# hkust-vgd/scanobjectnn

Measured on AMD Instinct MI355X. Metric: point-clouds/sec fwd+bwd at B×2048×3, 15-cls, higher is better.
Workload: dtype f32

## Files before the change

include/pcops.h:

```cpp
#ifndef PCOPS_H
#define PCOPS_H

#ifdef __cplusplus
extern "C" {
#endif

typedef void *pcops_stream_t;

typedef struct pcops_rows {
    const void *blocks;
    const int *block_start;
    const int *rows;
} pcops_rows_t;

typedef enum pcops_status {
    PCOPS_OK = 0,
    PCOPS_ERR_NULL_POINTER = -1,
    PCOPS_ERR_BAD_SHAPE = -2,
    PCOPS_ERR_BAD_ARGUMENT = -3,
    PCOPS_ERR_UNSUPPORTED = -4,
    PCOPS_ERR_LAUNCH = -5
} pcops_status;

const char *pcops_strerror(int status);
// ... 131 lines not shown
int pcops_mlp_wgrad_splits(long long M, int K, int N);
int pcops_mlp_wgrad(long long M, int K, int N, const float *X, int ldx, const float *a_scale,
                    const float *a_shift, const float *G, const float *Y, const float *p, const float *q,
                    const float *t, const float *gpool, const unsigned char *argmax, int S,
                    const float *pool_scale, const float *pool_shift, float *partial, float *dW, float *db,
                    pcops_stream_t stream);
int pcops_mlp_transpose(int K, int N, const float *W, float *Wt, pcops_stream_t stream);
int pcops_mlp_bwd_fused_groups(long long M, int K, int N, int S, int pooled);
int pcops_mlp_bwd_fused(long long M, int K, int N, const float *Yprev, const float *a_scale, const float *a_shift,
                        const float *G, const float *Y, const float *p, const float *q, const float *t,
                        const float *gpool, const unsigned char *argmax, int S, const float *W, float *partial,
                        float *dW, float *db, float *Gprev, float *stats_partial, pcops_stream_t stream);
int pcops_mlp_bwd_fused_rows(long long M, int K, int N, const float *Yprev, const float *a_scale, const float *a_shift,
                             const float *G, const float *Y, const float *p, const float *q, const float *t,
                             const float *gpool, const unsigned char *argmax, int S, const float *W, float *partial,
                             float *dW, float *db, float *Gprev, float *stats_partial, const pcops_rows_t *rows,
                             pcops_stream_t stream);
int pcops_mlp_dy_apply(long long M, int N, const float *G, const float *Y, const float *p, const float *q, const float *t,
                       float *out, pcops_stream_t stream);
int pcops_small_gemm(int M, int K, int N, const float *A, int lda, const float *B, int ldb, float *C, int ldc,
                     pcops_stream_t stream);
int pcops_small_gemm_ex(int M, int K, int N, const float *A, int lda, int transA, const float *B, int ldb, int transB,
                        const float *bias, float *C, int ldc, pcops_stream_t stream);
int pcops_small_gemm_colsum(int M, int K, int N, const float *A, int lda, int transA, const float *B, int ldb, int transB,
                            const float *bias, float *C, int ldc, float *colsum, pcops_stream_t stream);
typedef struct pcops_gemm_problem {
    int M, K, N;
    const float *A; int lda, transA;
    const float *B; int ldb, transB;
    const float *bias;
    float *C; int ldc;
    float *colsum;
} pcops_gemm_problem_t;
int pcops_small_gemm_pair(const pcops_gemm_problem_t *p, pcops_stream_t stream);

int pcops_mlp_pool_top_supported(int M, int Kp, int N, int S);
int pcops_mlp_pool_top_prep(int Kp, int N, const float *W, const float *b, const float *q, const float *t, float *Wt,
                            float *Wq, float *u, float *v, pcops_stream_t stream);
int pcops_mlp_pool_top_finish(int Kp, int N, long long M, float *dW, const float *Ssp, const float *xsum, const float *u,
                              const float *cfsum, const float *q, const float *W, const float *b, const float *t,
                              float *db, pcops_stream_t stream);
int pcops_mlp_pool_top_addend(int M, int Kp, int N, int S, const float *gout, const float *ysel,
                            const unsigned char *argmax, const float *pool_scale, const float *pool_shift,
                            const float *p, const float *Wt, float *addend, int *rowmap, pcops_stream_t stream);
int pcops_mlp_gemm_dgrad_top(int M, int Kp, const float *Yprev, const float *prev_scale, const float *prev_shift,
                             const float *Mq, const float *vconst, const float *addend, long long addend_rows,
                             const int *rowmap, float *Gprev, float *stats_partial, pcops_stream_t stream);
int pcops_mlp_gram(long long M, int Kp, const float *Yprev, int ldx, const float *a_scale, const float *a_shift,
                   float *partial, float *gram, float *xsum, pcops_stream_t stream);
int pcops_mlp_pool_top_wsparse(int M, int Kp, int N, int S, const float *gout, const float *ysel,
                               const unsigned char *argmax, const float *pool_scale, const float *pool_shift,
                               const float *p, const float *Yprev, const float *prev_scale, const float *prev_shift,
                               float *Ssp, float *cfsum, pcops_stream_t stream);
int pcops_mlp_xyz_supported(int M, int C1, int N2);
int pcops_mlp_bwd_fused_xyz_rows(long long M, int K, int N, const float *off4, const float *xyzw, const float *a_scale,
                                 const float *a_shift, const float *G, const float *Y, const float *p, const float *q,
                                 const float *t, const float *gpool, const unsigned char *argmax, int S, const float *W,
                                 float *partial, float *dW, float *db, float *stats_partial, float *xyz_stats,
                                 const pcops_rows_t *rows, pcops_stream_t stream);
int pcops_mlp_gemm_fwd_xyz(int M, int K, int N, const float *off4, const float *xyzw, const float *pro_scale,
                           const float *pro_shift, const float *W, const float *bias, float *Y,
                           float *stats_partial, const float *stat_pivot, pcops_stream_t stream);
int pcops_mlp_gemm_dgrad_xyz(int M, int K, int Nout, const float *G, const float *Y, const float *p,
                             const float *q, const float *t, const float *gpool, const unsigned char *argmax,
                             int S, const float *pool_scale, const float *pool_shift, const float *Wt,
                             const float *off4, const float *xyzw, const float *prev_scale,
                             const float *prev_shift, float *Gprev, float *stats_partial, float *xyz_stats,
                             pcops_stream_t stream);
int pcops_mlp_wgrad_xyz(long long M, int K, int N, const float *off4, const float *xyzw, const float *a_scale,
                        const float *a_shift, const float *G, const float *Y, const float *p, const float *q,
                        const float *t, const float *gpool, const unsigned char *argmax, int S,
                        const float *pool_scale, const float *pool_shift, float *partial, float *dW, float *db,
                        pcops_stream_t stream);

int pcops_sa_gather_stats_rows(long long groups);
int pcops_sa_gather_fwd_stats_rows(int b, int n, int m, int s, int c, int has_q, int has_ctr, int other_terms,
                                   int compacted);
int pcops_sa_gather_fwd(int b, int n, int m, int s, int c, const float *Q, const float *Ctr, const float *xyz,
                        const float *new_xyz, const float *Wxyz, const float *bias, const int *idx, float *Y,
                        float *off4, float *stats_partial, const float *stat_pivot, float *moments,
                        pcops_stream_t stream);
int pcops_sa_scatter_rows(int b, int m);
unsigned long long pcops_sa_scatter_workspace_bytes(int b, int n, int m, int s);
int pcops_sa_scatter_bwd(int b, int n, int m, int s, int c, const float *G, const float *Y, const float *p,
                         const float *q, const float *t, const float *gpool, const unsigned char *argmax,
                         const float *pool_scale, const float *pool_shift, const int *idx, const float *xyz,
                         const float *new_xyz, float *dQ, float *dCtr, float *wpartial, float *dWxyz,
                         float *dbias, const float *fwd_Q, const float *fwd_Ctr, const float *fwd_Wxyz,
                         const float *fwd_bias, void *workspace, pcops_stream_t stream);

int pcops_edge_pool_stats_rows(long long groups);
int pcops_edge_pool_fwd_stats_rows(int b, int n, int m, int s, int c);
int pcops_edge_pool_fwd(int b, int n, int m, int s, int c, const float *Q, const float *Ctr, const int *idx,
                        const float *gamma, float *SQ, float *qsel, unsigned char *arg, float *stats_partial,
                        const float *stat_pivot, pcops_stream_t stream);
int pcops_edge_pool_out(long long groups, int c, const float *qsel, const float *Ctr, const float *scale,
                        const float *shift, float *out, float *ysel, pcops_stream_t stream);
int pcops_edge_pool_bwd(int b, int n, int m, int s, int c, const float *Q, const float *Ctr, const int *idx,
                        const float *gpool, const float *ysel, const float *SQ, const unsigned char *arg,
                        const float *scale, const float *shift, const float *p, const float *q, const float *t,
                        float *dQ, float *dCtr, void *workspace, pcops_stream_t stream);
int pcops_cloud_bias_supported(long long rows, int rows_per_group, int c);
int pcops_cloud_bias_rows(long long rows);
int pcops_cloud_bias_fwd(long long rows, int rows_per_group, int c, const float *Q, const float *Ctr, float *Y,
                         float *stats_partial, const float *stat_pivot, pcops_stream_t stream);
int pcops_cloud_bias_bwd(long long rows, int rows_per_group, int c, const float *G, const float *Y, const float *p, const float *q,
// ... 223 lines not shown
```

scanobjectnn_amd/fused_mlp.py:

```python
import os
from collections import namedtuple
from typing import NamedTuple, Optional, Tuple

import torch

from . import _lib
from . import dist as _dist


def _f32(n, dev):
    return torch.empty(n, dtype=torch.float32, device=dev)


class _VecArena:

    def __init__(self, widths, per_width, dev):
        total = sum(((n + 3) // 4 * 4) * per_width for n in widths)
        alloc = torch.empty if all(n % 4 == 0 for n in widths) else torch.zeros
        self.buf = alloc(total, dtype=torch.float32, device=dev)
        self.off = 0

    def take(self, n):
        n4 = (n + 3) // 4 * 4
        v = self.buf[self.off:self.off + n4]
        self.off += n4
        return v


def _workspace(n, dev):
    lib = _lib.load()
    return torch.empty(int(lib.pcops_mlp_reduce_workspace_bytes(n)) // 8, dtype=torch.float64, device=dev)


def _p(t):
    return t.data_ptr() if t is not None else None


F_QC, F_CLOUD, F_GATHER, F_XYZ, F_POOL_ROWS, F_ROWS, F_POOL, F_GEMM = (
    "qc", "cloud_bias", "gather", "xyz", "pool_rows", "rows", "pool", "gemm")
F_CLOUD_POINT = "cloud_point"
B_XYZ_FIRST, B_EDGE_FIRST, B_QC, B_CLOUD, B_SCATTER, B_SCATTER_ID = (
    "xyz_first", "edge_first", "qc_scatter", "cloud_bias", "scatter", "scatter_identity")
B_CLOUD_POINT = "cloud_point"
B_TOP, B_SPLIT, B_SPLIT_XYZ = "top", "split", "split_xyz"
B_ONEPASS, B_ONEPASS_XYZ, B_ONEPASS_GW, B_ONEPASS_EDGE, B_ONEPASS_EDGE_GW = (
    "onepass", "onepass_xyz", "onepass_gw", "onepass_edge", "onepass_edge_gw")
_ONEPASS = (B_ONEPASS, B_ONEPASS_XYZ, B_ONEPASS_GW, B_ONEPASS_EDGE, B_ONEPASS_EDGE_GW)
_READS_Y = (B_CLOUD, B_CLOUD_POINT, B_SCATTER, B_SCATTER_ID, B_SPLIT, B_SPLIT_XYZ) + _ONEPASS
_READS_Y_BELOW = (B_TOP, B_SPLIT, B_ONEPASS, B_ONEPASS_GW, B_ONEPASS_EDGE, B_ONEPASS_EDGE_GW)


class LayerPlan(NamedTuple):
    fwd: str
    K: Optional[int]
    N: int
    store_y: bool
    pooled: str
    bwd: str
    count: int


class StackPlan(NamedTuple):
    virt: bool
    rows: bool
    direct: bool
    edge_rows: bool
    need_dx: bool
    tail_fold: bool
    layers: Tuple[LayerPlan, ...]

    @property
    def pool_top(self):
        return self.layers[-1].bwd == B_TOP


def plan_stack(*, R, S, K0, widths, pool, training, need_grad, need_dx, sync, w_aligned, has_b, geom=None, present=(),
               a0_contiguous=True, rows=False, point_k=None):
    lib = _lib.load()
    L, C1 = len(widths), widths[0]
    point = bool(pool & 16)
    identity, qc, direct, pool = bool(pool & 2), bool(pool & 4), bool(pool & 8), bool(pool & 1)
    gather = geom is not None
    direct = gather and qc and direct
    virt = (gather and "a0" not in present and "ctr" not in present and "wxyz" in present
            and (L >= 3 or (L == 2 and not pool)) and not sync and (training or not need_grad)
            and bool(lib.pcops_mlp_xyz_supported(R, C1, widths[1])))
    rows = rows and not (gather and "a0" not in present and not virt)
    edge_rows = False
    layers = []
    for l, N in enumerate(widths):
        K = widths[l - 1] if l else K0
        top = pool and l == L - 1
        store_y, pooled, bwd, count = True, "", "", 0
        onepass = int(need_grad and BWD_FUSED and l > 0 and lib.pcops_mlp_bwd_fused_groups(R, K, N, S if top else 0, int(top)))
        if l == 0 and gather:
            B, Nsrc, M = geom
            if point:
                if not (gather and identity and not qc and CLOUD_POINT_FUSED and set(present) == {"a0", "ctr", "wxyz"}
                        and not rows and not top and M == 1 and Nsrc == S and a0_contiguous and point_k is not None
                        and lib.pcops_cloud_point_supported(B, S, point_k, C1)):
                    raise _lib.PcopsError("plan_stack: no per-cloud + per-point first layer for this stack")
                fwd = F_CLOUD_POINT
            elif qc:
                fwd = F_QC
            elif (identity and CLOUD_BIAS and set(present) == {"a0", "ctr"} and not rows and M == 1 and Nsrc == S
                    and a0_contiguous and lib.pcops_cloud_bias_supported(R, S, C1)):
                fwd = F_CLOUD
            else:
                fwd, store_y = F_GATHER, not virt
            if need_grad:
                shortcut = "a0" in present and need_dx and identity and not top
                bwd = (B_CLOUD_POINT if fwd == F_CLOUD_POINT else B_XYZ_FIRST if virt else B_EDGE_FIRST if direct
                       else B_QC if qc else B_CLOUD if (fwd == F_CLOUD and not top) else B_SCATTER_ID if shortcut else B_SCATTER)
        else:
            xyz_prev = virt and l == 1
            algebraic = False
            if xyz_prev:
                fwd = F_XYZ
            elif rows and top and l > 0 and FUSE_POOL_ROWS and lib.pcops_mlp_gemm_fwd_pool_rows_supported(R, K, N):
                fwd, pooled = F_POOL_ROWS, "rows"
                algebraic = bool(need_grad and POOL_TOP and POOL_TOP_ROWS and S >= 64 and N >= 2 * K and has_b[l]
                                 and not onepass and lib.pcops_mlp_pool_top_rows_supported(R, K, N, S))
                store_y = not algebraic
            elif rows:
                fwd = F_ROWS
            elif top and lib.pcops_mlp_gemm_fwd_pool_supported(R, K, N, S):
                fwd, pooled = F_POOL, "raw"
                algebraic = bool(need_grad and POOL_TOP and S >= 64 and N >= 2 * K and has_b[l]
                                 and lib.pcops_mlp_pool_top_supported(R, K, N, S))
                store_y = need_grad and not algebraic
            else:
                fwd = F_GEMM
            if algebraic:
                bwd, count = B_TOP, lib.pcops_mlp_wgrad_splits(R, K, K)
            elif onepass and w_aligned[l]:
                use_edge = (direct and top and l == 1 and EDGE_DIRECT_FUSED
                            and lib.pcops_mlp_bwd_fused_edge_groups(R, K, N, S, 0) == onepass)
                gw = (top and not rows and not xyz_prev and
                      (lib.pcops_mlp_bwd_fused_edge_groups(R, K, N, S, 1) if use_edge
                       else lib.pcops_mlp_bwd_fused_gw_groups(R, K, N, S)) == onepass)
                edge_rows = edge_rows or use_edge
                bwd = ((B_ONEPASS_EDGE_GW if gw else B_ONEPASS_EDGE) if use_edge else B_ONEPASS_GW if gw
                       else B_ONEPASS_XYZ if xyz_prev else B_ONEPASS)
                count = onepass
            elif need_grad:
                bwd, count = (B_SPLIT_XYZ if xyz_prev else B_SPLIT), lib.pcops_mlp_wgrad_splits(R, K, N)
        layers.append(LayerPlan(fwd, K, N, bool(store_y), pooled, bwd, int(count)))
    for l, lp in enumerate(layers):
        reads = (lp.bwd in _READS_Y or (l + 1 < L and layers[l + 1].bwd in _READS_Y_BELOW)
                 or (need_grad and not pool and l == L - 1))
        assert lp.store_y or not reads, (l, layers)
    return StackPlan(bool(virt), bool(rows), direct, bool(edge_rows), bool(need_dx), TAIL_FOLD, tuple(layers))


StackSaved = namedtuple("StackSaved", "a0 ctr idx xyz new_xyz wxyz bias Ys means rstds scales shifts Ws gammas argmax ysel "
                                      "off4 xyzw mom")


def _bn_forward(bn, N, R, P, part, piv, *, training, sync, need_grad, hyper, vecs, ws):
    (gamma, beta, mm, mv), (eps, decay, unbiased) = bn, hyper
    scale, shift = vecs.take(N), vecs.take(N)
    mean = rstd = None
    if training:
        mean, rstd = vecs.take(N), vecs.take(N)
        Pf, Rf, piv_fin = P, R, piv
        if sync:
            part, Rf = _dist.allreduce_stat_partials(part, R, mm if piv is not None else None)
            Pf, piv_fin = part.shape[0], None
        _lib.call("pcops_mlp_bn_finalize", Pf, N, Rf, part.data_ptr(), piv_fin, ws.data_ptr(), gamma.data_ptr(),
                  beta.data_ptr(), float(eps), float(decay), int(unbiased), mm.data_ptr(), mv.data_ptr(),
                  mean.data_ptr(), rstd.data_ptr(), scale.data_ptr(), shift.data_ptr())
    else:
        _lib.call("pcops_mlp_bn_eval_coeffs", N, gamma.data_ptr(), beta.data_ptr(), mm.data_ptr(),
                  mv.data_ptr(), float(eps), scale.data_ptr(), shift.data_ptr())
        if need_grad:
            mean, rstd = mm.detach().clone(), torch.rsqrt(mv.detach() + float(eps))
    return scale, shift, mean, rstd


def _bn_backward(N, R, P, part, gamma, mean, rstd, *, training, sync, vecs, ws):
    dev = part.device
    dgamma, dbeta = _f32(N, dev), _f32(N, dev)
    p, q, t = vecs.take(N), vecs.take(N), vecs.take(N)
    _lib.call("pcops_mlp_bn_bwd_coeffs", P, N, R, part.data_ptr(), ws.data_ptr(), gamma.data_ptr(),
              mean.data_ptr(), rstd.data_ptr(), dgamma.data_ptr(), dbeta.data_ptr(),
              p.data_ptr(), q.data_ptr(), t.data_ptr())
    if sync:
        gpart, Rg = _dist.allreduce_stat_partials(part, R)
        junk = _f32(2 * N, dev)
        _lib.call("pcops_mlp_bn_bwd_coeffs", gpart.shape[0], N, Rg, gpart.data_ptr(), ws.data_ptr(), gamma.data_ptr(),
                  mean.data_ptr(), rstd.data_ptr(), junk.data_ptr(), junk[N:].data_ptr(),
                  p.data_ptr(), q.data_ptr(), t.data_ptr())
    if not training:
        q.zero_()
        t.zero_()
    return dgamma, dbeta, p, q, t


class FusedMLPStack(torch.autograd.Function):

# ... 419 lines not shown
                  S, psc, psh, scratch.data_ptr(), dW.data_ptr(), db.data_ptr(), rref)
    else:
        src, asc, ash = (sv.Ys[l - 1], sv.scales[l - 1].data_ptr(), sv.shifts[l - 1].data_ptr()) if l else (sv.a0, None, None)
        _lib.call("pcops_mlp_wgrad_rows", R, K, N, src.data_ptr(), K, asc, ash, Gptr, Y.data_ptr(),
                  p.data_ptr(), q.data_ptr(), t.data_ptr(), gp, am, S, psc, psh, scratch.data_ptr(),
                  dW.data_ptr(), db.data_ptr(), rref)
    dn.grads[6 * l + 0] = dW
    dn.grads[6 * l + 1] = db
    if l == 0 and not dn.plan.need_dx:
        return
    Wt = _f32((N, K), dev)
    _lib.call("pcops_mlp_transpose", K, N, sv.Ws[l].data_ptr(), Wt.data_ptr())
    Gprev = None if xyz_prev else _f32((R, K), dev)
    if l > 0:
        dn.P = lib.pcops_mlp_stats_rows(R)
        dn.part = _f32((dn.P, 2, K), dev)
    if xyz_prev:
        dn.xstats = _f32((dn.P, 3, K), dev)
        _lib.call("pcops_mlp_gemm_dgrad_xyz_rows", R, N, K, Gptr, Y.data_ptr(), p.data_ptr(), q.data_ptr(),
                  t.data_ptr(), gp, am, S, psc, psh, Wt.data_ptr(), sv.off4.data_ptr(), sv.xyzw.data_ptr(),
                  sv.scales[0].data_ptr(), sv.shifts[0].data_ptr(), None, dn.part.data_ptr(), dn.xstats.data_ptr(),
                  rref)
    elif l > 0:
        _lib.call("pcops_mlp_gemm_dgrad_rows", R, N, K, Gptr, Y.data_ptr(), p.data_ptr(), q.data_ptr(),
                  t.data_ptr(), gp, am, S, psc, psh, Wt.data_ptr(), sv.Ys[l - 1].data_ptr(),
                  sv.scales[l - 1].data_ptr(), sv.shifts[l - 1].data_ptr(), Gprev.data_ptr(),
                  dn.part.data_ptr(), rref)
    else:
        _lib.call("pcops_mlp_gemm_dgrad", R, N, K, Gptr, Y.data_ptr(), p.data_ptr(), q.data_ptr(),
                  t.data_ptr(), gp, am, S, psc, psh, Wt.data_ptr(), None, None, None,
                  Gprev.data_ptr(), None)
    dn.Gm = Gprev


def _pool_top_backward(dn, l, lp, p, q, t):
    lib = _lib.load()
    sv, dev, R, S, rows, rref = dn.sv, dn.dev, dn.R, dn.S, dn.rows, dn.rref
    K, N, fold = lp.K, lp.N, dn.plan.tail_fold
    W, b, grad_out = sv.Ws[l], dn.biases[l].detach(), dn.grad_out
    ysel, argmax, sc, sh = sv.ysel, sv.argmax, sv.scales[l], sv.shifts[l]
    Yprev, psc, psh = (sv.Ys[l - 1], sv.scales[l - 1], sv.shifts[l - 1]) if l > 0 else (sv.a0, None, None)
    need_dx = l > 0 or dn.plan.need_dx
    Wt = _f32((N, K), dev)
    if fold:
        Wq, u = _f32((K, N), dev), _f32(N, dev)
        v = _f32(K, dev) if need_dx else None
        _lib.call("pcops_mlp_pool_top_prep", K, N, W.data_ptr(), b.data_ptr(), q.data_ptr(), t.data_ptr(), Wt.data_ptr(),
                  Wq.data_ptr(), u.data_ptr(), _p(v))
    else:
        _lib.call("pcops_mlp_transpose", K, N, W.data_ptr(), Wt.data_ptr())
        Wq = W * q[:N]
        u = torch.addcmul(t[:N], q[:N], b)
    Gprev = part = None
    scratch = _f32(lp.count * (K * K + K), dev)
    gram, xsum = _f32((K, K), dev), _f32(K, dev)
    if rows is not None:
        _lib.call("pcops_mlp_gram_rows", R, K, Yprev.data_ptr(), K, _p(psc), _p(psh), scratch.data_ptr(),
                  gram.data_ptr(), xsum.data_ptr(), rref)
    else:
        _lib.call("pcops_mlp_gram", R, K, Yprev.data_ptr(), K, _p(psc), _p(psh), scratch.data_ptr(),
                  gram.data_ptr(), xsum.data_ptr())
    dW = _f32((K, N), dev)
    paired = fold and need_dx
    if paired:
        Mq = _f32((K, K), dev)
        _lib.small_gemm_pair((K, N, K, Wq.data_ptr(), N, 0, Wt.data_ptr(), K, 0, None, Mq.data_ptr(), K, None),
                             (K, K, N, gram.data_ptr(), K, 0, Wq.data_ptr(), N, 0, None, dW.data_ptr(), N, None))
    if need_dx:
        if not paired:
            Mq = _f32((K, K), dev)
            _lib.call("pcops_small_gemm", K, N, K, Wq.data_ptr(), N, Wt.data_ptr(), K, Mq.data_ptr(), K)
        if not fold:
            v = _f32(K, dev)
            _lib.call("pcops_small_gemm", 1, N, K, u.data_ptr(), N, Wt.data_ptr(), K, v.data_ptr(), K)
        G = R // S
        addend = _f32((R if rows is not None else G * min(S, N), K), dev)
        rowmap = torch.empty(R, dtype=torch.int32, device=dev)
        Gprev = _f32((R, K), dev)
        part = _f32((lib.pcops_mlp_stats_rows(R), 2, K), dev) if psc is not None else None
        if rows is not None:
            _lib.call("pcops_mlp_pool_top_addend_rows", R, K, N, S, grad_out.data_ptr(), ysel.data_ptr(),
                      argmax.data_ptr(), sc.data_ptr(), sh.data_ptr(), p.data_ptr(), Wt.data_ptr(), addend.data_ptr(),
                      rowmap.data_ptr(), rref)
            _lib.call("pcops_mlp_gemm_dgrad_top_rows", R, K, Yprev.data_ptr(), _p(psc), _p(psh), Mq.data_ptr(),
                      v.data_ptr(), addend.data_ptr(), addend.shape[0], rowmap.data_ptr(), Gprev.data_ptr(), _p(part),
                      rref)
        else:
            _lib.call("pcops_mlp_pool_top_addend", R, K, N, S, grad_out.data_ptr(), ysel.data_ptr(), argmax.data_ptr(),
                      sc.data_ptr(), sh.data_ptr(), p.data_ptr(), Wt.data_ptr(), addend.data_ptr(), rowmap.data_ptr())
            _lib.call("pcops_mlp_gemm_dgrad_top", R, K, Yprev.data_ptr(), _p(psc), _p(psh), Mq.data_ptr(),
                      v.data_ptr(), addend.data_ptr(), addend.shape[0], rowmap.data_ptr(), Gprev.data_ptr(), _p(part))
    Ssp, cfsum = _f32((K, N), dev), _f32(N, dev)
    if rows is not None:
        wpart = _f32(int(lib.pcops_mlp_pool_top_wsparse_rows_partial(K, N)), dev)
        _lib.call("pcops_mlp_pool_top_wsparse_rows", R, K, N, S, grad_out.data_ptr(), ysel.data_ptr(), argmax.data_ptr(),
                  sc.data_ptr(), sh.data_ptr(), p.data_ptr(), Yprev.data_ptr(), _p(psc), _p(psh),
                  Ssp.data_ptr(), cfsum.data_ptr(), wpart.data_ptr(), rref)
    else:
        _lib.call("pcops_mlp_pool_top_wsparse", R, K, N, S, grad_out.data_ptr(), ysel.data_ptr(), argmax.data_ptr(),
                  sc.data_ptr(), sh.data_ptr(), p.data_ptr(), Yprev.data_ptr(), _p(psc), _p(psh),
                  Ssp.data_ptr(), cfsum.data_ptr())
    if not paired:
        _lib.call("pcops_small_gemm", K, K, N, gram.data_ptr(), K, Wq.data_ptr(), N, dW.data_ptr(), N)
    if fold:
        db = _f32(N, dev)
        _lib.call("pcops_mlp_pool_top_finish", K, N, R, dW.data_ptr(), Ssp.data_ptr(), xsum.data_ptr(), u.data_ptr(),
                  cfsum.data_ptr(), q.data_ptr(), W.data_ptr(), b.data_ptr(), t.data_ptr(), db.data_ptr())
        dn.grads[6 * l + 0] = dW
        dn.grads[6 * l + 1] = db
    else:
        xw = _f32(N, dev)
        _lib.call("pcops_small_gemm", 1, K, N, xsum.data_ptr(), K, W.data_ptr(), N, xw.data_ptr(), N)
        dn.grads[6 * l + 0] = torch.addr(dW.add_(Ssp), xsum, u)
        dn.grads[6 * l + 1] = cfsum + q[:N] * (xw + float(R) * b) + float(R) * t[:N]
    dn.Gm, dn.P, dn.part = Gprev, lib.pcops_mlp_stats_rows(R), part


class _SmallLinear(torch.autograd.Function):

    @staticmethod
    def forward(ctx, x, w, b):
        R, K = x.shape
        N = w.shape[1]
        y = torch.empty((R, N), dtype=torch.float32, device=x.device)
        _lib.call("pcops_small_gemm_ex", R, K, N, x.data_ptr(), K, 0, w.data_ptr(), N, 0, _p(b), y.data_ptr(), N)
        ctx.save_for_backward(x, w)
        ctx.has_bias = b is not None
        return y

    @staticmethod
    @torch.autograd.function.once_differentiable
    def backward(ctx, gy):
        x, w = ctx.saved_tensors
        R, K = x.shape
        N = w.shape[1]
        gy = gy.contiguous()
        dx = dw = db = None
        want_db = ctx.has_bias and ctx.needs_input_grad[2]
        if TAIL_FOLD and ctx.needs_input_grad[0] and ctx.needs_input_grad[1]:
            dx = torch.empty((R, K), dtype=torch.float32, device=x.device)
            dw = torch.empty((K, N), dtype=torch.float32, device=x.device)
            db = torch.empty(N, dtype=torch.float32, device=x.device) if want_db else None
            _lib.small_gemm_pair((R, N, K, gy.data_ptr(), N, 0, w.data_ptr(), N, 1, None, dx.data_ptr(), K, None),
                                 (K, R, N, x.data_ptr(), K, 1, gy.data_ptr(), N, 0, None, dw.data_ptr(), N, _p(db)))
            return dx, dw, db
        if ctx.needs_input_grad[0]:
            dx = torch.empty((R, K), dtype=torch.float32, device=x.device)
            _lib.call("pcops_small_gemm_ex", R, N, K, gy.data_ptr(), N, 0, w.data_ptr(), N, 1, None, dx.data_ptr(), K)
        if ctx.needs_input_grad[1]:
            dw = torch.empty((K, N), dtype=torch.float32, device=x.device)
            if want_db and TAIL_FOLD:
# ... 329 lines not shown
            dQC = _f32((B, Nsrc, 2 * C), dev)
            _lib.call("pcops_edge_pool_bwd_ld", B, Nsrc, M, S, C, Q.data_ptr(), 2 * C, Q.data_ptr() + 4 * C, 2 * C,
                      idx.data_ptr(), grad_out.data_ptr(), ysel.data_ptr(), SQ.data_ptr(), arg.data_ptr(), scale.data_ptr(),
                      shift.data_ptr(), p.data_ptr(), q.data_ptr(), t.data_ptr(), dQC.data_ptr(), 2 * C,
                      dQC.data_ptr() + 4 * C, 2 * C, wsp.data_ptr())
            return dQC, None, None, dgamma, dbeta, None, None, None, None, None, None, None, None
        dQ, dCtr = _f32((B, Nsrc, C), dev), _f32((B, M, C), dev)
        _lib.call("pcops_edge_pool_bwd", B, Nsrc, M, S, C, Q.data_ptr(), Ctr.data_ptr(), idx.data_ptr(),
                  grad_out.data_ptr(), ysel.data_ptr(), SQ.data_ptr(), arg.data_ptr(), scale.data_ptr(), shift.data_ptr(),
                  p.data_ptr(), q.data_ptr(), t.data_ptr(), dQ.data_ptr(), dCtr.data_ptr(), wsp.data_ptr())
        return dQ, dCtr, None, dgamma, dbeta, None, None, None, None, None, None, None, None


def edge_conv_pool_supported(C, S):
    return C in (32, 64, 128) or C % 256 == 0 and S <= 256


def fused_supported(x, widths, bn, activation_relu):
    if not (bn and activation_relu and x.is_cuda and x.dtype == torch.float32):
        return False
    if any(w % 32 != 0 for w in widths):
        return False
    return True


def _flat(layer_tensors, first_gather):
    flat = []
    for i, (w, b, gamma, beta, mm, mv) in enumerate(layer_tensors):
        if i == 0 and first_gather:
            flat.extend([None, None, gamma, beta, mm, mv])
        else:
            flat.extend([w.reshape(-1, w.shape[-1]), b, gamma, beta, mm, mv])
    return flat


def mlp_stack(x, S, pool, training, decay, eps, unbiased, layer_tensors):
    x2d = x.reshape(-1, x.shape[-1]).contiguous()
    return FusedMLPStack.apply(x2d, None, None, None, None, None, None, int(S), bool(pool), bool(training),
                               float(decay), float(eps), bool(unbiased), None, len(layer_tensors),
                               *_flat(layer_tensors, False))


TRACE = None
STAT_PIVOT = os.environ.get("PCOPS_STAT_PIVOT", "1") != "0"
FUSE_POOL_ROWS = os.environ.get("PCOPS_FUSE_POOL_ROWS", "1") != "0"
BWD_FUSED = os.environ.get("PCOPS_BWD_FUSED", "1") != "0"
CLOUD_BIAS = os.environ.get("PCOPS_CLOUD_BIAS", "1") != "0"
CLOUD_POINT = os.environ.get("PCOPS_CLOUD_POINT", "1") != "0"
CLOUD_POINT_FUSED = os.environ.get("PCOPS_CLOUD_POINT_FUSED", "1") != "0"
EDGE_DIRECT = os.environ.get("PCOPS_EDGE_DIRECT", "1") != "0"
EDGE_DIRECT_FUSED = os.environ.get("PCOPS_EDGE_DIRECT_FUSED", "1") != "0"
POOL_TOP = os.environ.get("PCOPS_POOL_TOP", "1") != "0"
POOL_TOP_ROWS = os.environ.get("PCOPS_POOL_TOP_ROWS", "1") != "0"
TAIL_FOLD = os.environ.get("PCOPS_TAIL_FOLD", "1") != "0"
COMPACT_MIN_S = int(os.environ.get("PCOPS_COMPACT_MIN_S", "48"))
EDGE_QC = os.environ.get("PCOPS_EDGE_QC", "1") != "0"


def _compactable(idx, pool, L, widths, Q, Ctr, xyz, wxyz, identity_idx):
    B, M, S = idx.shape
    if not (COMPACT_MIN_S and pool and not identity_idx and Ctr is None and L >= 2 and S >= COMPACT_MIN_S):
        return False
    if B * M * S < 32768 or any(w % 32 for w in widths) or _dist.sync_bn_active():
        return False
    if Q is None and not (wxyz is not None and L >= 3):
        return False
    import ctypes
    n = Q.shape[1] if Q is not None else xyz.shape[1]
    arr = (ctypes.c_int * L)(*[int(w) for w in widths])
    return bool(_lib.load().pcops_gather_stack_rows_supported(B, n, M, S, 1 if Q is not None else 0, L, arr))


def edge_qc_supported(b, n, s, c):
    return bool(EDGE_QC and _lib.load().pcops_edge_ld_supported(int(b), int(n), int(n), int(s), int(c))
                and not _dist.sync_bn_active())


def cloud_point_fused_supported(b, n, k, c1):
    return bool(CLOUD_POINT_FUSED and _lib.load().pcops_cloud_point_supported(int(b), int(n), int(k), int(c1)))


def edge_direct_supported(b, n, k, c_in, c1, n_layers, x):
    if not (EDGE_DIRECT and c_in == 3 and n_layers >= 2) or (torch.is_grad_enabled() and x.requires_grad):
        return False
    return bool(_lib.load().pcops_edge_first_supported(b, n, n, k, c1))


def gather_mlp_stack(idx, pool, training, decay, eps, unbiased, layer_tensors, Q=None, Ctr=None, xyz=None,
                     new_xyz=None, wxyz=None, bias=None, identity_idx=False, pts_cnt=None, QC=None, cat_slot=None,
                     direct=None, point=None):
    c = lambda t: t.contiguous() if t is not None else None
    S = idx.shape[2]
    if point is not None:
        x64, wx = point
        assert QC is None and Q is None and xyz is None and wxyz is None and bias is None and identity_idx and not pool
        return FusedMLPStack.apply(x64.contiguous(), c(Ctr), idx.contiguous(), None, None, wx.contiguous(), None, int(S),
                                   2 | 16, bool(training), float(decay), float(eps), bool(unbiased), None,
                                   len(layer_tensors), *_flat(layer_tensors, True))
    if QC is not None:
        assert Q is None and Ctr is None and xyz is None and wxyz is None and bias is None
        if len(layer_tensors) == 1 and pool:
            _w, _b, gamma, beta, mm, mv = layer_tensors[0]
            if cat_slot is not None:
                return EdgeConvPool.apply(QC.contiguous(), None, idx.contiguous(), gamma, beta, mm, mv, bool(training),
                                          float(decay), float(eps), bool(unbiased), cat_slot[0], int(cat_slot[1]))
            return EdgeConvPool.apply(QC.contiguous(), None, idx.contiguous(), gamma, beta, mm, mv, bool(training),
# ... 28 lines not shown
```

Baseline: 26930.

## Add fused group-tiled pool-top backward kernels for small-S pooled layers

```diff
diff --git a/include/pcops.h b/include/pcops.h
--- a/include/pcops.h
+++ b/include/pcops.h
@@ -207,6 +207,17 @@
                                const unsigned char *argmax, const float *pool_scale, const float *pool_shift,
                                const float *p, const float *Yprev, const float *prev_scale, const float *prev_shift,
                                float *Ssp, float *cfsum, pcops_stream_t stream);
+int pcops_mlp_pool_top_groups_supported(int M, int Kp, int N, int S);
+int pcops_mlp_pool_top_groups_partial(int M, int Kp, int N);
+int pcops_mlp_dgrad_top_groups(int M, int Kp, int N, int S, const float *Yprev, const float *prev_scale,
+                               const float *prev_shift, const float *Mq, const float *vconst, const float *gout,
+                               const float *ysel, const unsigned char *argmax, const float *pool_scale,
+                               const float *pool_shift, const float *p, const float *Wt, float *Gprev, float *stats_partial,
+                               pcops_stream_t stream);
+int pcops_mlp_wgrad_top_groups(int M, int Kp, int N, int S, const float *Yprev, const float *prev_scale,
+                               const float *prev_shift, const float *gout, const float *ysel, const unsigned char *argmax,
+                               const float *pool_scale, const float *pool_shift, const float *p, float *partial, float *gram,
+                               float *xsum, float *Ssp, float *cfsum, pcops_stream_t stream);
 int pcops_mlp_xyz_supported(int M, int C1, int N2);
 int pcops_mlp_bwd_fused_xyz_rows(long long M, int K, int N, const float *off4, const float *xyzw, const float *a_scale,
                                  const float *a_shift, const float *G, const float *Y, const float *p, const float *q,
diff --git a/scanobjectnn_amd/csrc/pooltop_groups.hip b/scanobjectnn_amd/csrc/pooltop_groups.hip
--- /dev/null
+++ b/scanobjectnn_amd/csrc/pooltop_groups.hip
@@ -0,0 +1,403 @@
+#include "common.h"
+
+namespace {
+
+typedef float f32x16 __attribute__((ext_vector_type(16)));
+
+constexpr int KP = 64;
+constexpr int TR = 64;
+constexpr int XLD = KP + 4;
+constexpr int NMAX = 256;
+constexpr int MW = NMAX / 32;
+constexpr unsigned kOOB32 = 0x7FFFFFF0u;
+constexpr int kMaxGrid = 512;
+
+struct TileRegs {
+    float4 y[4];
+    float go[2], ys[2];
+    int am[2];
+};
+template <bool ROWS> __device__ __forceinline__ int trow(int i) { return ROWS ? (int)(threadIdx.x >> 2) : 16 * i + (int)(threadIdx.x >> 4); }
+template <bool ROWS> __device__ __forceinline__ int tcol(int i) { return ROWS ? 4 * ((int)(threadIdx.x & 3) + 4 * i) : 4 * (int)(threadIdx.x & 15); }
+
+template <bool ROWS>
+__device__ __forceinline__ void tile_request(TileRegs &t, long long tile, long long ntiles, long long M, long long G, int N,
+                                             int gpt, const float *__restrict__ Yprev, const float *__restrict__ gout,
+                                             const float *__restrict__ ysel, const unsigned char *__restrict__ arg) {
+    const int tid = threadIdx.x;
+    const long long tl = tile < ntiles ? tile : ntiles - 1;
+#pragma unroll
+    for (int j = 0; j < 2; ++j) {
+        const int e = tid + 256 * j;
+        const int gl = e / N;
+        const long long g = tl * gpt + (gl < gpt ? gl : 0);
+        const long long o = (g < G ? g : G - 1) * N + (e - gl * N);
+        t.go[j] = gout[o]; t.ys[j] = ysel[o]; t.am[j] = arg[o];
+    }
+#pragma unroll
+    for (int i = 0; i < 4; ++i) {
+        const long long r = tl * TR + trow<ROWS>(i);
+        t.y[i] = *reinterpret_cast<const float4 *>(Yprev + (r < M ? r : M - 1) * KP + tcol<ROWS>(i));
+    }
+}
+
+__device__ __forceinline__ float triple_cf(const TileRegs &t, int j, long long tile, long long G, int N, int gpt,
+                                           const float *pv) {
+    const int e = threadIdx.x + 256 * j, gl = e / N, c = e - gl * N;
+    if (gl >= gpt || tile * gpt + gl >= G) return 0.f;
+    return fmaf(t.ys[j], pv[c], pv[NMAX + c]) > 0.f ? pv[2 * NMAX + c] * t.go[j] : 0.f;
+}
+
+__device__ __forceinline__ float4 bn_relu4(float4 y, float4 sc, float4 sh, bool in) {
+    float4 x;
+    x.x = in ? fmaxf(fmaf(y.x, sc.x, sh.x), 0.f) : 0.f;
+    x.y = in ? fmaxf(fmaf(y.y, sc.y, sh.y), 0.f) : 0.f;
+    x.z = in ? fmaxf(fmaf(y.z, sc.z, sh.z), 0.f) : 0.f;
+    x.w = in ? fmaxf(fmaf(y.w, sc.w, sh.w), 0.f) : 0.f;
+    return x;
+}
+
+constexpr int WLD = KP + 4;
+
+__global__ __launch_bounds__(256) void dgrad_top_groups_kernel(long long M, int N, int S, const float *__restrict__ Yprev,
+                                                               const float *__restrict__ psc, const float *__restrict__ psh,
+                                                               const float *__restrict__ Mq, const float *__restrict__ vconst,
+                                                               const float *__restrict__ gout, const float *__restrict__ ysel,
+                                                               const unsigned char *__restrict__ arg,
+                                                               const float *__restrict__ sc, const float *__restrict__ sh,
+                                                               const float *__restrict__ p, const float *__restrict__ Wt,
+                                                               float *__restrict__ Gprev, float *__restrict__ stats) {
+    extern __shared__ __attribute__((aligned(16))) float lds[];
+    float *wts = lds;
+    float *xs = wts + N * WLD;
+    float *os = xs + TR * XLD;
+    float *cst = os + TR * XLD;
+    float *cfl = cst + 3 * KP;
+    float *pv = cfl + 2 * NMAX;
+    unsigned *mask = reinterpret_cast<unsigned *>(pv + 3 * NMAX);
+    const int tid = threadIdx.x, lane = tid & 63, wave = tid >> 6, row = tid >> 2, qj = tid & 3;
+    const int gpt = TR / S, nw2 = (N + 63) / 64;
+    const long long G = M / S, ntiles = (M + TR - 1) / TR;
+
+    for (int i = tid; i < N * KP / 4; i += 256)
+        *reinterpret_cast<float4 *>(wts + (i >> 4) * WLD + 4 * (i & 15)) = reinterpret_cast<const float4 *>(Wt)[i];
+    for (int i = tid; i < TR * MW; i += 256) mask[i] = 0u;
+    if (tid < KP) { cst[tid] = psc[tid]; cst[KP + tid] = psh[tid]; cst[2 * KP + tid] = vconst[tid]; }
+    if (tid < N) { pv[tid] = sc[tid]; pv[NMAX + tid] = sh[tid]; pv[2 * NMAX + tid] = p[tid]; }
+    const int l32 = lane & 31, h = lane >> 5, row0 = 32 * (wave >> 1), col0 = 32 * (wave & 1);
+    float bq[32];
+#pragma unroll
+    for (int j = 0; j < 8; ++j)
+#pragma unroll
+        for (int e = 0; e < 4; ++e) bq[4 * j + e] = Mq[(8 * j + 4 * h + e) * KP + col0 + l32];
+    float4 s1[4], s2[4];
+#pragma unroll
+    for (int k = 0; k < 4; ++k) s1[k] = s2[k] = make_float4(0.f, 0.f, 0.f, 0.f);
+
+    const float *cfg = cfl + (row / S) * NMAX;
+    const float *wrow = wts + 4 * qj;
+    unsigned long long *mrow = reinterpret_cast<unsigned long long *>(mask + row * MW);
+    auto do_tile = [&](long long tile, TileRegs &cur, TileRegs &nxt) {
+        tile_request<true>(nxt, tile + gridDim.x, ntiles, M, G, N, gpt, Yprev, gout, ysel, arg);
+        const bool in = tile * TR + row < M;
+#pragma unroll
+        for (int k = 0; k < 4; ++k) {
+            const int c = tcol<true>(k);
+            *reinterpret_cast<float4 *>(xs + row * XLD + c) =
+                bn_relu4(cur.y[k], *reinterpret_cast<const float4 *>(cst + c), *reinterpret_cast<const float4 *>(cst + KP + c), in);
+        }
+#pragma unroll
+        for (int j = 0; j < 2; ++j) {
+            const int e = tid + 256 * j, gl = e / N, c = e - gl * N;
+            if (gl < gpt) {
+                const float cf = triple_cf(cur, j, tile, G, N, gpt, pv);
+                cfl[gl * NMAX + c] = cf;
+                if (cf != 0.f && cur.am[j] < S) atomicOr(&mask[(gl * S + cur.am[j]) * MW + (c >> 5)], 1u << (c & 31));
+            }
+        }
+        __syncthreads();
+        f32x16 acc = {0.f, 0.f, 0.f, 0.f, 0.f, 0.f, 0.f, 0.f, 0.f, 0.f, 0.f, 0.f, 0.f, 0.f, 0.f, 0.f};
+#pragma unroll
+        for (int j = 0; j < 8; ++j) {
+            const float4 a = *reinterpret_cast<const float4 *>(xs + (row0 + l32) * XLD + 8 * j + 4 * h);
+            acc = __builtin_amdgcn_mfma_f32_32x32x2f32(a.x, bq[4 * j + 0], acc, 0, 0, 0);
+            acc = __builtin_amdgcn_mfma_f32_32x32x2f32(a.y, bq[4 * j + 1], acc, 0, 0, 0);
+            acc = __builtin_amdgcn_mfma_f32_32x32x2f32(a.z, bq[4 * j + 2], acc, 0, 0, 0);
+            acc = __builtin_amdgcn_mfma_f32_32x32x2f32(a.w, bq[4 * j + 3], acc, 0, 0, 0);
+        }
+#pragma unroll
+        for (int i = 0; i < 16; ++i)
+            os[(row0 + 8 * (i >> 2) + 4 * h + (i & 3)) * XLD + col0 + l32] = acc[i];
+        float4 add[4];
+#pragma unroll
+        for (int k = 0; k < 4; ++k) add[k] = make_float4(0.f, 0.f, 0.f, 0.f);
+        for (int w2 = 0; w2 < nw2; ++w2) {
+            unsigned long long m = mrow[w2];
+            if (qj == 0) mrow[w2] = 0ull;
+            int c = m ? 64 * w2 + __builtin_ctzll(m) : 0;
+            float cfn = m ? cfg[c] : 0.f;
+            float4 wn[4];
+#pragma unroll
+            for (int k = 0; k < 4; ++k) wn[k] = *reinterpret_cast<const float4 *>(wrow + c * WLD + 16 * k);
+            while (m) {
+                m &= m - 1;
+                const float cf = cfn;
+                float4 wc[4];
+#pragma unroll
+                for (int k = 0; k < 4; ++k) wc[k] = wn[k];
+                c = m ? 64 * w2 + __builtin_ctzll(m) : 0;
+                cfn = m ? cfg[c] : 0.f;
+#pragma unroll
+                for (int k = 0; k < 4; ++k) wn[k] = *reinterpret_cast<const float4 *>(wrow + c * WLD + 16 * k);
+#pragma unroll
+                for (int k = 0; k < 4; ++k) {
+                    add[k].x = fmaf(cf, wc[k].x, add[k].x); add[k].y = fmaf(cf, wc[k].y, add[k].y);
+                    add[k].z = fmaf(cf, wc[k].z, add[k].z); add[k].w = fmaf(cf, wc[k].w, add[k].w);
+                }
+            }
+        }
+        __syncthreads();
+        if (in) {
+            float *dst = Gprev + (tile * TR + row) * KP;
+#pragma unroll
+            for (int k = 0; k < 4; ++k) {
+                const int c = tcol<true>(k);
+                const float4 o = *reinterpret_cast<const float4 *>(os + row * XLD + c);
+                const float4 vsc = *reinterpret_cast<const float4 *>(cst + c), vsh = *reinterpret_cast<const float4 *>(cst + KP + c);
+                const float4 vc = *reinterpret_cast<const float4 *>(cst + 2 * KP + c);
+                const float4 y = cur.y[k];
+                float4 d;
+                d.x = fmaf(y.x, vsc.x, vsh.x) > 0.f ? (o.x + vc.x) + add[k].x : 0.f;
+                d.y = fmaf(y.y, vsc.y, vsh.y) > 0.f ? (o.y + vc.y) + add[k].y : 0.f;
+                d.z = fmaf(y.z, vsc.z, vsh.z) > 0.f ? (o.z + vc.z) + add[k].z : 0.f;
+                d.w = fmaf(y.w, vsc.w, vsh.w) > 0.f ? (o.w + vc.w) + add[k].w : 0.f;
+                *reinterpret_cast<float4 *>(dst + c) = d;
+                s1[k].x += d.x; s1[k].y += d.y; s1[k].z += d.z; s1[k].w += d.w;
+                s2[k].x = fmaf(d.x, y.x, s2[k].x); s2[k].y = fmaf(d.y, y.y, s2[k].y);
+                s2[k].z = fmaf(d.z, y.z, s2[k].z); s2[k].w = fmaf(d.w, y.w, s2[k].w);
+            }
+        }
+    };
+    TileRegs ra, rb;
+    tile_request<true>(ra, blockIdx.x, ntiles, M, G, N, gpt, Yprev, gout, ysel, arg);
+    __syncthreads();
+    for (long long tile = blockIdx.x; tile < ntiles; tile += 2 * gridDim.x) {
+        do_tile(tile, ra, rb);
+        if (tile + gridDim.x < ntiles) do_tile(tile + gridDim.x, rb, ra);
+    }
+    __syncthreads();
+    float *red = xs;
+#pragma unroll
+    for (int k = 0; k < 4; ++k) {
+        *reinterpret_cast<float4 *>(red + (row * 2 + 0) * KP + tcol<true>(k)) = s1[k];
+        *reinterpret_cast<float4 *>(red + (row * 2 + 1) * KP + tcol<true>(k)) = s2[k];
+    }
+    __syncthreads();
+    if (tid < 2 * KP) {
+        float s = 0.f;
+        for (int i = 0; i < TR; ++i) s += red[i * 2 * KP + tid];
+        stats[(long long)blockIdx.x * 2 * KP + tid] = s;
+    }
+}
+
+template <int KS>
+__global__ __launch_bounds__(256) void wgrad_top_groups_kernel(long long M, int N, int S, const float *__restrict__ Yprev,
+                                                               const float *__restrict__ psc, const float *__restrict__ psh,
+                                                               const float *__restrict__ gout, const float *__restrict__ ysel,
+                                                               const unsigned char *__restrict__ arg,
+                                                               const float *__restrict__ sc, const float *__restrict__ sh,
+                                                               const float *__restrict__ p, float *__restrict__ partial) {
+    constexpr int KW = KP / KS;
+    __shared__ __attribute__((aligned(16))) float xs[TR * XLD];
+    __shared__ float cfl[2 * NMAX];
+    __shared__ int aml[2 * NMAX];
+    __shared__ float pv[3 * NMAX];
+    const int tid = threadIdx.x, lane = tid & 63, wave = tid >> 6, rr = tid >> 4, q = tid & 15;
+    const int gpt = TR / S;
+    const long long G = M / S, ntiles = (M + TR - 1) / TR;
+    const int l32 = lane & 31, h = lane >> 5;
+    const int cch = KS == 2 ? (tid & 127) : tid, k0 = KS == 2 ? 32 * (tid >> 7) : 0;
+    const float4 vsc = *reinterpret_cast<const float4 *>(psc + 4 * q), vsh = *reinterpret_cast<const float4 *>(psh + 4 * q);
+
+    f32x16 g00 = {0.f, 0.f, 0.f, 0.f, 0.f, 0.f, 0.f, 0.f, 0.f, 0.f, 0.f, 0.f, 0.f, 0.f, 0.f, 0.f}, g01 = g00, g11 = g00;
+    float4 xsum = make_float4(0.f, 0.f, 0.f, 0.f);
+    float sp[KW];
+#pragma unroll
+    for (int k = 0; k < KW; ++k) sp[k] = 0.f;
+    float cfs = 0.f;
+
+    if (tid < N) { pv[tid] = sc[tid]; pv[NMAX + tid] = sh[tid]; pv[2 * NMAX + tid] = p[tid]; }
+    __syncthreads();
+    TileRegs cur, nxt;
+    tile_request<false>(cur, blockIdx.x, ntiles, M, G, N, gpt, Yprev, gout, ysel, arg);
+    for (long long tile = blockIdx.x; tile < ntiles; tile += gridDim.x) {
+        tile_request<false>(nxt, tile + gridDim.x, ntiles, M, G, N, gpt, Yprev, gout, ysel, arg);
+#pragma unroll
+        for (int i = 0; i < 4; ++i) {
+            const float4 x = bn_relu4(cur.y[i], vsc, vsh, tile * TR + 16 * i + rr < M);
+            *reinterpret_cast<float4 *>(xs + (16 * i + rr) * XLD + 4 * q) = x;
+            xsum.x += x.x; xsum.y += x.y; xsum.z += x.z; xsum.w += x.w;
+        }
+#pragma unroll
+        for (int j = 0; j < 2; ++j) {
+            const int e = tid + 256 * j, gl = e / N, c = e - gl * N;
+            if (gl < gpt) {
+                cfl[gl * NMAX + c] = triple_cf(cur, j, tile, G, N, gpt, pv);
+                aml[gl * NMAX + c] = cur.am[j] < S ? cur.am[j] : S - 1;
+            }
+        }
+        __syncthreads();
+#pragma unroll
+        for (int st = 0; st < 8; ++st) {
+            const float *xr = xs + (16 * wave + 2 * st + h) * XLD;
+            const float f0 = xr[l32], f1 = xr[32 + l32];
+            g00 = __builtin_amdgcn_mfma_f32_32x32x2f32(f0, f0, g00, 0, 0, 0);
+            g01 = __builtin_amdgcn_mfma_f32_32x32x2f32(f0, f1, g01, 0, 0, 0);
+            g11 = __builtin_amdgcn_mfma_f32_32x32x2f32(f1, f1, g11, 0, 0, 0);
+        }
+        for (int gl = 0; gl < gpt; ++gl) {
+            const float cf = cch < N ? cfl[gl * NMAX + cch] : 0.f;
+            const float *xr = xs + (gl * S + (cch < N ? aml[gl * NMAX + cch] : 0)) * XLD + k0;
+#pragma unroll
+            for (int k = 0; k < KW; k += 4) {
+                const float4 x = *reinterpret_cast<const float4 *>(xr + k);
+                sp[k + 0] = fmaf(cf, x.x, sp[k + 0]); sp[k + 1] = fmaf(cf, x.y, sp[k + 1]);
+                sp[k + 2] = fmaf(cf, x.z, sp[k + 2]); sp[k + 3] = fmaf(cf, x.w, sp[k + 3]);
+            }
+            cfs += cf;
+        }
+        __syncthreads();
+        cur = nxt;
+    }
+    float *part = partial + (long long)blockIdx.x * (KP * KP + KP + KP * N + N);
+    float *pg = part, *px = pg + KP * KP, *ps = px + KP, *pc = ps + KP * N;
+    float *red = xs;
+    for (int w = 0; w < 4; ++w) {
+        if (wave == w) {
+#pragma unroll
+            for (int i = 0; i < 16; ++i) {
+                const int o = (8 * (i >> 2) + 4 * h + (i & 3)) * 32 + l32;
+                if (w == 0) { red[o] = g00[i]; red[1024 + o] = g01[i]; red[2048 + o] = g11[i]; }
+                else { red[o] += g00[i]; red[1024 + o] += g01[i]; red[2048 + o] += g11[i]; }
+            }
+        }
+        __syncthreads();
+    }
+    for (int i = tid; i < KP * KP; i += 256) {
+        const int r = i >> 6, c = i & 63;
+        const int br = r >> 5, bc = c >> 5;
+        float v;
+        if (br <= bc) v = red[(br + bc) * 1024 + (r & 31) * 32 + (c & 31)];
+        else v = red[1024 + (c & 31) * 32 + (r & 31)];
+        pg[i] = v;
+    }
+    __syncthreads();
+    *reinterpret_cast<float4 *>(red + rr * KP + 4 * q) = xsum;
+    __syncthreads();
+    if (tid < KP) {
+        float s = 0.f;
+#pragma unroll
+        for (int i = 0; i < 16; ++i) s += red[i * KP + tid];
+        px[tid] = s;
+    }
+    if (cch < N) {
+#pragma unroll
+        for (int k = 0; k < KW; ++k) ps[(k0 + k) * N + cch] = sp[k];
+        if (k0 == 0) pc[cch] = cfs;
+    }
+}
+
+__global__ __launch_bounds__(1024) void groups_sum_kernel(int P, int L, int N, const float *__restrict__ part,
+                                                          float *__restrict__ gram, float *__restrict__ xsum,
+                                                          float *__restrict__ Ssp, float *__restrict__ cfsum) {
+    __shared__ double sm[16][64];
+    const int c = threadIdx.x & 63, pl = threadIdx.x >> 6;
+    const int i = blockIdx.x * 64 + c;
+    double s = 0.0;
+    if (i < L)
+        for (int pp = pl; pp < P; pp += 16) s += (double)part[(long long)pp * L + i];
+    sm[pl][c] = s;
+    __syncthreads();
+    if (pl == 0 && i < L) {
+        double t = 0.0;
+#pragma unroll
+        for (int k = 0; k < 16; ++k) t += sm[k][c];
+        const int o1 = KP * KP, o2 = o1 + KP, o3 = o2 + KP * N;
+        float *dst = i < o1 ? gram + i : i < o2 ? xsum + (i - o1) : i < o3 ? Ssp + (i - o2) : cfsum + (i - o3);
+        *dst = (float)t;
+    }
+}
+
+bool groups_shape_ok(long long M, int Kp, int N, int S) {
+    return Kp == KP && N % 32 == 0 && N >= 64 && N <= NMAX && N >= 2 * Kp && (S == 32 || S == 64) && M >= S && M % S == 0 &&
+           M * Kp * 4 < (long long)kOOB32;
+}
+
+int groups_grid(long long M) {
+    const long long ntiles = (M + TR - 1) / TR;
+    return (int)(ntiles < kMaxGrid ? ntiles : kMaxGrid);
+}
+
+bool aligned16(const void *ptr) { return (reinterpret_cast<uintptr_t>(ptr) & 15) == 0; }
+
+}
+
+extern "C" {
+
+int pcops_mlp_stats_rows(int M);
+
+int pcops_mlp_pool_top_groups_supported(int M, int Kp, int N, int S) {
+    return groups_shape_ok(M, Kp, N, S) && M >= 262144 ? 1 : 0;
+}
+
+int pcops_mlp_pool_top_groups_partial(int M, int Kp, int N) {
+    if (M < 1 || Kp != KP || N < 1 || N > NMAX) return 0;
+    return groups_grid(M) * (Kp * Kp + Kp + Kp * N + N);
+}
+
+int pcops_mlp_dgrad_top_groups(int M, int Kp, int N, int S, const float *Yprev, const float *prev_scale,
+                               const float *prev_shift, const float *Mq, const float *vconst, const float *gout,
+                               const float *ysel, const unsigned char *argmax, const float *pool_scale,
+                               const float *pool_shift, const float *p, const float *Wt, float *Gprev, float *stats_partial,
+                               pcops_stream_t stream) {
+    if (!groups_shape_ok(M, Kp, N, S)) return PCOPS_ERR_UNSUPPORTED;
+    PCOPS_REQUIRE_PTR(Yprev); PCOPS_REQUIRE_PTR(prev_scale); PCOPS_REQUIRE_PTR(prev_shift); PCOPS_REQUIRE_PTR(Mq);
+    PCOPS_REQUIRE_PTR(vconst); PCOPS_REQUIRE_PTR(gout); PCOPS_REQUIRE_PTR(ysel); PCOPS_REQUIRE_PTR(argmax);
+    PCOPS_REQUIRE_PTR(pool_scale); PCOPS_REQUIRE_PTR(pool_shift); PCOPS_REQUIRE_PTR(p); PCOPS_REQUIRE_PTR(Wt);
+    PCOPS_REQUIRE_PTR(Gprev); PCOPS_REQUIRE_PTR(stats_partial);
+    if (!aligned16(Yprev) || !aligned16(prev_scale) || !aligned16(prev_shift) || !aligned16(vconst) || !aligned16(Wt) ||
+        !aligned16(Gprev))
+        return PCOPS_ERR_UNSUPPORTED;
+    const int grid = pcops_mlp_stats_rows(M);
+    if (grid < 1 || grid > kMaxGrid || grid > (M + TR - 1) / TR) return PCOPS_ERR_UNSUPPORTED;
+    const size_t lds = (size_t)(N * WLD + 2 * TR * XLD + 3 * KP + 5 * NMAX + TR * MW) * sizeof(float);
+    pcops_note_pipe(0);
+    return pcops_launch_lds(dgrad_top_groups_kernel, dim3(grid), dim3(256), lds, 160 * 1024, as_stream(stream), (long long)M, N,
+                            S, Yprev, prev_scale, prev_shift, Mq, vconst, gout, ysel, argmax, pool_scale, pool_shift, p, Wt,
+                            Gprev, stats_partial);
+}
+
+int pcops_mlp_wgrad_top_groups(int M, int Kp, int N, int S, const float *Yprev, const float *prev_scale,
+                               const float *prev_shift, const float *gout, const float *ysel, const unsigned char *argmax,
+                               const float *pool_scale, const float *pool_shift, const float *p, float *partial, float *gram,
+                               float *xsum, float *Ssp, float *cfsum, pcops_stream_t stream) {
+    if (!groups_shape_ok(M, Kp, N, S)) return PCOPS_ERR_UNSUPPORTED;
+    PCOPS_REQUIRE_PTR(Yprev); PCOPS_REQUIRE_PTR(prev_scale); PCOPS_REQUIRE_PTR(prev_shift); PCOPS_REQUIRE_PTR(gout);
+    PCOPS_REQUIRE_PTR(ysel); PCOPS_REQUIRE_PTR(argmax); PCOPS_REQUIRE_PTR(pool_scale); PCOPS_REQUIRE_PTR(pool_shift);
+    PCOPS_REQUIRE_PTR(p); PCOPS_REQUIRE_PTR(partial); PCOPS_REQUIRE_PTR(gram); PCOPS_REQUIRE_PTR(xsum); PCOPS_REQUIRE_PTR(Ssp);
+    PCOPS_REQUIRE_PTR(cfsum);
+    if (!aligned16(Yprev) || !aligned16(prev_scale) || !aligned16(prev_shift)) return PCOPS_ERR_UNSUPPORTED;
+    hipStream_t st = as_stream(stream);
+    const int grid = groups_grid(M), L = Kp * Kp + Kp + Kp * N + N;
+    pcops_note_pipe(0);
+    if (N <= 128)
+        hipLaunchKernelGGL(wgrad_top_groups_kernel<2>, dim3(grid), dim3(256), 0, st, (long long)M, N, S, Yprev, prev_scale,
+                           prev_shift, gout, ysel, argmax, pool_scale, pool_shift, p, partial);
+    else
+        hipLaunchKernelGGL(wgrad_top_groups_kernel<1>, dim3(grid), dim3(256), 0, st, (long long)M, N, S, Yprev, prev_scale,
+                           prev_shift, gout, ysel, argmax, pool_scale, pool_shift, p, partial);
+    hipLaunchKernelGGL(groups_sum_kernel, dim3(cdiv(L, 64)), dim3(1024), 0, st, grid, L, N, partial, gram, xsum, Ssp, cfsum);
+    return pcops_launch_status();
+}
+
+}
diff --git a/scanobjectnn_amd/fused_mlp.py b/scanobjectnn_amd/fused_mlp.py
--- a/scanobjectnn_amd/fused_mlp.py
+++ b/scanobjectnn_amd/fused_mlp.py
@@ -58,6 +58,7 @@
     pooled: str
     bwd: str
     count: int
+    groups: bool = False
 
 
 class StackPlan(NamedTuple):
@@ -115,6 +116,7 @@
         else:
             xyz_prev = virt and l == 1
             algebraic = False
+            groups = False
             if xyz_prev:
                 fwd = F_XYZ
             elif rows and top and l > 0 and FUSE_POOL_ROWS and lib.pcops_mlp_gemm_fwd_pool_rows_supported(R, K, N):
@@ -128,6 +130,9 @@
                 fwd, pooled = F_POOL, "raw"
                 algebraic = bool(need_grad and POOL_TOP and S >= 64 and N >= 2 * K and has_b[l]
                                  and lib.pcops_mlp_pool_top_supported(R, K, N, S))
+                groups = bool(need_grad and POOL_TOP and POOL_TOP_GROUPS and l > 0 and has_b[l] and w_aligned[l]
+                              and lib.pcops_mlp_pool_top_groups_supported(R, K, N, S))
+                algebraic = algebraic or groups
                 store_y = need_grad and not algebraic
             else:
                 fwd = F_GEMM
@@ -145,7 +150,7 @@
                 count = onepass
             elif need_grad:
                 bwd, count = (B_SPLIT_XYZ if xyz_prev else B_SPLIT), lib.pcops_mlp_wgrad_splits(R, K, N)
-        layers.append(LayerPlan(fwd, K, N, bool(store_y), pooled, bwd, int(count)))
+        layers.append(LayerPlan(fwd, K, N, bool(store_y), pooled, bwd, int(count), bool(bwd == B_TOP and groups)))
     for l, lp in enumerate(layers):
         reads = (lp.bwd in _READS_Y or (l + 1 < L and layers[l + 1].bwd in _READS_Y_BELOW)
                  or (need_grad and not pool and l == L - 1))
@@ -671,12 +676,20 @@
         Wq = W * q[:N]
         u = torch.addcmul(t[:N], q[:N], b)
     Gprev = part = None
-    scratch = _f32(lp.count * (K * K + K), dev)
     gram, xsum = _f32((K, K), dev), _f32(K, dev)
-    if rows is not None:
+    Ssp, cfsum = _f32((K, N), dev), _f32(N, dev)
+    if lp.groups:
+        wpart = _f32(int(lib.pcops_mlp_pool_top_groups_partial(R, K, N)), dev)
+        _lib.call("pcops_mlp_wgrad_top_groups", R, K, N, S, Yprev.data_ptr(), psc.data_ptr(), psh.data_ptr(),
+                  grad_out.data_ptr(), ysel.data_ptr(), argmax.data_ptr(), sc.data_ptr(), sh.data_ptr(), p.data_ptr(),
+                  wpart.data_ptr(), gram.data_ptr(), xsum.data_ptr(), Ssp.data_ptr(), cfsum.data_ptr())
+        del wpart
+    elif rows is not None:
+        scratch = _f32(lp.count * (K * K + K), dev)
         _lib.call("pcops_mlp_gram_rows", R, K, Yprev.data_ptr(), K, _p(psc), _p(psh), scratch.data_ptr(),
                   gram.data_ptr(), xsum.data_ptr(), rref)
     else:
+        scratch = _f32(lp.count * (K * K + K), dev)
         _lib.call("pcops_mlp_gram", R, K, Yprev.data_ptr(), K, _p(psc), _p(psh), scratch.data_ptr(),
                   gram.data_ptr(), xsum.data_ptr())
     dW = _f32((K, N), dev)
@@ -693,11 +706,15 @@
             v = _f32(K, dev)
             _lib.call("pcops_small_gemm", 1, N, K, u.data_ptr(), N, Wt.data_ptr(), K, v.data_ptr(), K)
         G = R // S
-        addend = _f32((R if rows is not None else G * min(S, N), K), dev)
-        rowmap = torch.empty(R, dtype=torch.int32, device=dev)
         Gprev = _f32((R, K), dev)
         part = _f32((lib.pcops_mlp_stats_rows(R), 2, K), dev) if psc is not None else None
-        if rows is not None:
+        if lp.groups:
+            _lib.call("pcops_mlp_dgrad_top_groups", R, K, N, S, Yprev.data_ptr(), psc.data_ptr(), psh.data_ptr(),
+                      Mq.data_ptr(), v.data_ptr(), grad_out.data_ptr(), ysel.data_ptr(), argmax.data_ptr(), sc.data_ptr(),
+                      sh.data_ptr(), p.data_ptr(), Wt.data_ptr(), Gprev.data_ptr(), part.data_ptr())
+        elif rows is not None:
+            addend = _f32((R, K), dev)
+            rowmap = torch.empty(R, dtype=torch.int32, device=dev)
             _lib.call("pcops_mlp_pool_top_addend_rows", R, K, N, S, grad_out.data_ptr(), ysel.data_ptr(),
                       argmax.data_ptr(), sc.data_ptr(), sh.data_ptr(), p.data_ptr(), Wt.data_ptr(), addend.data_ptr(),
                       rowmap.data_ptr(), rref)
@@ -705,17 +722,18 @@
                       v.data_ptr(), addend.data_ptr(), addend.shape[0], rowmap.data_ptr(), Gprev.data_ptr(), _p(part),
                       rref)
         else:
+            addend = _f32((G * min(S, N), K), dev)
+            rowmap = torch.empty(R, dtype=torch.int32, device=dev)
             _lib.call("pcops_mlp_pool_top_addend", R, K, N, S, grad_out.data_ptr(), ysel.data_ptr(), argmax.data_ptr(),
                       sc.data_ptr(), sh.data_ptr(), p.data_ptr(), Wt.data_ptr(), addend.data_ptr(), rowmap.data_ptr())
             _lib.call("pcops_mlp_gemm_dgrad_top", R, K, Yprev.data_ptr(), _p(psc), _p(psh), Mq.data_ptr(),
                       v.data_ptr(), addend.data_ptr(), addend.shape[0], rowmap.data_ptr(), Gprev.data_ptr(), _p(part))
-    Ssp, cfsum = _f32((K, N), dev), _f32(N, dev)
-    if rows is not None:
+    if rows is not None and not lp.groups:
         wpart = _f32(int(lib.pcops_mlp_pool_top_wsparse_rows_partial(K, N)), dev)
         _lib.call("pcops_mlp_pool_top_wsparse_rows", R, K, N, S, grad_out.data_ptr(), ysel.data_ptr(), argmax.data_ptr(),
                   sc.data_ptr(), sh.data_ptr(), p.data_ptr(), Yprev.data_ptr(), _p(psc), _p(psh),
                   Ssp.data_ptr(), cfsum.data_ptr(), wpart.data_ptr(), rref)
-    else:
+    elif not lp.groups:
         _lib.call("pcops_mlp_pool_top_wsparse", R, K, N, S, grad_out.data_ptr(), ysel.data_ptr(), argmax.data_ptr(),
                   sc.data_ptr(), sh.data_ptr(), p.data_ptr(), Yprev.data_ptr(), _p(psc), _p(psh),
                   Ssp.data_ptr(), cfsum.data_ptr())
@@ -1151,6 +1169,7 @@
 EDGE_DIRECT_FUSED = os.environ.get("PCOPS_EDGE_DIRECT_FUSED", "1") != "0"
 POOL_TOP = os.environ.get("PCOPS_POOL_TOP", "1") != "0"
 POOL_TOP_ROWS = os.environ.get("PCOPS_POOL_TOP_ROWS", "1") != "0"
+POOL_TOP_GROUPS = os.environ.get("PCOPS_POOL_TOP_GROUPS", "1") != "0"
 TAIL_FOLD = os.environ.get("PCOPS_TAIL_FOLD", "1") != "0"
 COMPACT_MIN_S = int(os.environ.get("PCOPS_COMPACT_MIN_S", "48"))
 EDGE_QC = os.environ.get("PCOPS_EDGE_QC", "1") != "0"
```

New measurement: 27300 (median of 6 runs). 1.01x the previous value.
